# ende76/brotli-rs

Measured on AMD Instinct MI355X. Metric: decompressed MB/s (whole node), alice29x4096 batch, higher is better.
Workload: dtype u8; 1 GPU; 4096 x alice29.txt.compressed per GPU; streams_per_gpu=4096

## Files before the change

### brotli-rs_amd/csrc/brx_hot.S

```

#include "brx_layout.h"
#define RMASK 2047
#define RING BRX_L_RING_BYTES
#define LDS_TM BRX_L_TM
#define LDS_ST BRX_L_ST
#define LDS_MBW BRX_L_MBW
#define LDS_ITAB BRX_L_ITAB
#define LDS_SPARE BRX_L_SPARE
#define LDS_CMH BRX_L_CMH
#define LDS_PAD0 BRX_L_PAD
#define SYMOFF 68
#define INFOOFF 64
#define XLOOP 0x1ffff

#define NPOST s4
#define MA s5
#define MB s6
#define SB s7
#define PFREE s8
#define PBASE s9
#define DTREE s10
#define LINKD s[24:25]
#define XFP s[26:27]
#define LITSYM s28
// ... 10 lines not shown
#define DIST s47
#define RSRC s[48:51]
#define RSRC2 s[16:19]
#define POS s52
#define DSPEC s57
#define SKEW s53
#define VFL s54
#define FLUSHAT s55
#define WINDOW s56
#define INS s92
#define CPY s93
#define MBLEFT s61
#define IZ s64
#define LBLEN s65
#define IBLEN s66
#define DBLEN s67
#define PRIOW s60
#define RUN s68
#define NXT s[58:59]
#define NXTLO s58
#define NXTHI s59
#define WIN s[62:63]
#define WINLO s62
#define WINHI s63
#define MBEND s69
#ifdef BRX_WIN_SGPR
#define SNAV s70
#else
#define SWC s70
#endif
#define DCTX s94
#define HISYM s71
#define MA2 s71
#define BFEB s28
#define CMDW s72
#define EXITC s73
#define IACTAB s[74:75]
#define DICTP s[76:77]
#define LBLEN_REAL s78
#define IBLEN_REAL s79
#define FLAGS s80
#define DCODE s81
#define LINKA s[82:83]
#define T0 s84
#define T1 s85
#define T01 s[84:85]
#define T2 s86
#define T3 s87
#define T4 s88
#define T5 s89
#define T6 s90
#define T7 s91
#define CLEN s96
#if defined(BRX_WIN_SGPR) && !defined(BRX_PROF) && !defined(BRX_NO_SLOTS)
#define BRX_SLOTS
#endif
#ifndef SLOT_OVER
#define SLOT_OVER 11
#endif
#ifndef BRX_PROF
#define LITJ s[20:21]
#define LITJLO s20
#define LITJHI s21
#ifdef BRX_SLOTS
#define BFEBI s29
#define VCCB s[22:23]
#define VCCA s[30:31]
// ... 150 lines not shown
.endm
.macro TAKE_EXTRA dst, base, n, rid, mul=0
    v_bfe_u32 VEX, VWINLO, 0, \n
    .ifnc \mul,0
    v_mad_u32_u24 VEX, VEX, \mul, \base
    .else
    v_add_u32 VEX, \base, VEX
    .endif
    TAKE \n, \rid
    v_readfirstlane_b32 \dst, VEX
.endm
.macro REFILL_CORE
    v_readlane_b32 T0, VCHA, WL
    v_mov_b32 VWLO, VWHI
    s_sub_u32 SWC, SWC, 32
    s_add_u32 WL, WL, 1
    v_mov_b32 VWHI, T0
    s_cmp_lg_u32 WL, WLSTOP
.endm
.macro WIN_INIT lo, hi
    v_mov_b32 VWLO, \lo
    v_mov_b32 VWHI, \hi
    v_alignbit_b32 VWINLO, VWHI, VWLO, SWC
.endm
.macro WIN_ROLLED
.endm
#endif
#ifndef STUB_PAD_NOPS
#define STUB_PAD_NOPS 5
#endif
#ifndef TAIL_PAD_NOPS
#define TAIL_PAD_NOPS 0
#endif
.macro STUB_PAD
#ifndef BRX_WIN_SGPR
    .rept STUB_PAD_NOPS
    s_nop 0
    .endr
#endif
.endm
.macro REFILL_STUB id
.Lrf_stub_\id:
    REFILL_CORE
    s_cbranch_scc1 .Lrf_back_\id
    s_call_b64 LINKA, .Lspecial
    s_branch .Lrf_back_\id
    STUB_PAD
.endm
.macro TO_COUNTS reg, tmp
    v_add_u32 \tmp, -1, VSH
    v_lshrrev_b32 \reg, \tmp, \reg
.endm
.macro SPLIT_TREE lim, base
    v_bfe_i32 \base, \lim, 0, 16
    v_and_b32 \lim, 0xffff0000, \lim
.endm
.macro LOOKUP lim, base
    v_bfrev_b32 VR, WSRC
    v_lshrrev_b32 VU, 1, VR
    v_cmp_lt_u32 vcc, VU, \lim
    s_ff1_i32_b32 CLEN, vcc_lo
    v_readlane_b32 T3, \base, CLEN
    s_sub_u32 T2, 32, CLEN
    v_lshrrev_b32 VI, T2, VR
    v_add_u32 VI, T3, VI
.endm

#ifdef BRX_NO_SPEC
.macro LOOKUP2 lim, base, symbase, scale, rd, off, rid
    v_bfrev_b32 VR, WSRC
    v_lshrrev_b32 VU, 1, VR
    v_cmp_lt_u32 vcc, VU, \lim
    s_ff1_i32_b32 CLEN, vcc_lo
// ... 403 lines not shown
    s_cbranch_scc1 .Lent_multi
    s_bitset1_b32 FLAGS, 3
    s_add_u32 LITSYM, T6, SYMOFF
    v_add_u32 VT0, T6, VLANE4
    ds_read_b32 VLITL, VT0
.Lent_multi:
    s_waitcnt vmcnt(0)
    v_readlane_b32 s36, VCHA, 0
    v_readlane_b32 s37, VCHA, 1
#ifdef BRX_WIN_SGPR
    s_lshr_b64 s[36:37], s[36:37], T3
    s_sub_u32 SNAV, 32, T3
#else
    s_sub_u32 SWC, T3, 32
#endif
    WIN_INIT s36, s37
    s_mov_b32 WL, 2
    s_sub_u32 T0, WSAFE, CBASE
    s_cselect_b32 T0, 0, T0
    s_min_u32 WLSTOP, T0, 64
#ifdef BRX_PROF
    s_mov_b32 s20, 0
    s_mov_b32 s21, 0
    s_mov_b32 s22, 0
    s_mov_b32 s23, 0
    s_mov_b32 s29, 0
    s_mov_b32 s30, 0
    s_mov_b32 s31, 0
    s_memtime s[12:13]
    s_memtime s[16:17]
    s_waitcnt lgkmcnt(0)
#endif
    s_mov_b32 PFREE, 0
    s_mov_b32 PBASE, POS
    s_sub_u32 DCTX, CPY, 2
    s_min_u32 DCTX, DCTX, 3
    s_cmp_lg_u32 IZ, 0
    s_cselect_b32 DCTX, 4, DCTX
    s_mov_b32 T0, 0xc0000000
    s_lshl_b32 DCTX, DCTX, 1
    v_writelane_b32 VDH4, T0, 8
#ifdef BRX_DIST_RESIDENT
    s_call_b64 LINKB, .Lload_dtrees
#endif
    s_mov_b32 EXITC, 1
    s_and_b32 T0, VFL, 0xfffffc00
    s_add_u32 T0, T0, 1024
    s_sub_u32 FLUSHAT, T0, SKEW
    s_waitcnt lgkmcnt(0)
    s_cmp_lt_u32 WLSTOP, 3
    s_cbranch_scc1 .Lexit
    s_and_b32 T0, VFL, 1023
    s_cmp_lg_u32 T0, 0
    s_cbranch_scc1 .Lexit
    SPLIT_TREE VIACL, VIACB
    SPLIT_TREE VLITL, VLITB
    v_lshl_add_u32 VIACB, VIACB, 1, HISYM
    v_lshl_add_u32 VLITB, VLITB, 1, LITSYM
    TO_COUNTS VIACL, VT3
    TO_COUNTS VLITL, VT3
    s_lshr_b32 MA2, MA, 2
    s_mov_b32 BFEB, 0
    s_cmp_eq_u32 SB, 2
    s_cselect_b32 BFEB, 0x20008, BFEB
    s_cmp_eq_u32 MB, 0x1c
    s_cselect_b32 BFEB, 0x3000a, BFEB
#ifndef BRX_PROF
    s_sub_u32 BFEBI, BFEB, 8
    s_cmp_eq_u32 BFEB, 0
    s_cselect_b32 BFEBI, 0, BFEBI
    s_getpc_b64 LITJ
.Llitj_base:
    s_mov_b32 T0, .Llit_entry_g-.Llitj_base
    s_bitcmp1_b32 FLAGS, 5
    s_cselect_b32 T0, .Llit_r_entry_mx-.Llitj_base, T0
    s_cselect_b32 T1, 0x1c, -1
    s_cmp_eq_u32 T1, MB
    s_cselect_b32 T0, .Llit_r_entry_m3-.Llitj_base, T0
#ifdef BRX_SLOTS
    s_bitcmp1_b32 FLAGS, 6
    s_cselect_b32 T0, .Llit_r_entry_sx-.Llitj_base, T0
    s_cselect_b32 T1, 0x1c, -1
    s_cmp_eq_u32 T1, MB
    s_cselect_b32 T0, .Llit_r_entry_s3-.Llitj_base, T0
#endif
    s_bitcmp1_b32 FLAGS, 3
    s_cselect_b32 T0, .Lhave_lits1-.Llitj_base, T0
    s_add_u32 LITJLO, LITJLO, T0
    s_addc_u32 LITJHI, LITJHI, 0
#endif
    s_mov_b32 MAXA, 0
    s_mov_b64 exec, XLOOP
    s_branch .Lr1
// ... 67 lines not shown
    s_waitcnt lgkmcnt(0)
    v_readlane_b32 DCODE, VS, CLEN
    s_cmp_lt_i32 DCODE, 0
    s_cbranch_scc1 .Ldist_ring
    s_and_b32 T1, DCODE, 31
#ifdef BRX_WIN_SGPR
    s_lshr_b32 T2, DCODE, 5
    TAKE_EXTRA DIST, T2, T1, 6, NPOST
#else
    v_lshrrev_b32 VT0, 5, DCODE
    TAKE_EXTRA DIST, VT0, T1, 6, NPOST
#endif
.Ldist_push:
    PROF_MARK s30
    s_cmp_gt_u32 DIST, MAXA
    s_cbranch_scc1 .Ldict_check
.Ldist_push_ok:
    v_mov_b32_dpp VRING, VRING row_shr:1 row_mask:0xf bank_mask:0xf
    v_writelane_b32 VRING, DIST, 0

.Lcopy:
#ifndef BRX_NO_SPEC
    LOOKUP2F_EARLY VIACL, VIACB, 1, ds_read_u16
#endif
    s_bfm_b64 exec, CPY, PFREE
    s_add_u32 PFREE, PFREE, CPY
    s_min_u32 T0, DIST, 63
    s_cmp_gt_u32 PFREE, T0
    s_cbranch_scc1 .Lcopy_slow_undo
    s_sub_u32 T2, PBASE, DIST
    s_cmp_gt_u32 DIST, RING
    s_cbranch_scc0 .Lcopy_near
    v_add_u32 VT0, T2, VLANE
    buffer_load_ubyte VPEND, VT0, RSRC, 0 offen
    s_mov_b64 exec, XLOOP
    s_add_u32 POS, POS, CPY
.Lcopy_tail_pre:
    s_cmp_ge_u32 POS, MBEND
    s_cbranch_scc0 .Lcmd_pre
    s_branch .Lcopy_end
.Lcopy_tail:
.Lflush_back_cmd:
    s_cmp_ge_u32 POS, MBEND
    s_cbranch_scc0 .Lcmd
.Lcopy_end:
    s_cmp_eq_u32 POS, MBEND
    s_cbranch_scc0 .Lcopy_overrun
    s_mov_b32 INS, 0
    s_branch .Lexit
.Lcopy_overrun:
    s_sub_u32 POS, POS, CPY
    s_sub_u32 PFREE, PFREE, CPY
    s_branch .Lx_r2

.Lcopy_near:
    s_add_u32 T2, T2, SKEW
    v_add_u32 VT0, T2, VLANE
    v_and_b32 VT0, RMASK, VT0
    ds_read_u8 VPEND, VT0
    s_mov_b64 exec, XLOOP
    s_add_u32 POS, POS, CPY
    s_cmp_ge_u32 POS, MBEND
    s_cbranch_scc0 .Lcmd_pre
    s_branch .Lcopy_end

#ifdef BRX_DIST_RESIDENT
.Ldist_other:
    s_add_u32 T0, DCTX, 16
    s_bitcmp1_b32 DSPEC, T0
    s_cbranch_scc1 .Ldist_special
    s_sub_u32 DBLEN, DBLEN, 1
    s_cbranch_scc1 .Lx_dist_switch
.Ldist_ticked:
    v_bfrev_b32 VR, WSRC
    v_lshrrev_b32 VI, VSH, VR
    s_set_gpr_idx_on DCTX, 6
    v_cmp_lt_u32 vcc, VI, VDTREES
    v_lshl_add_u32 VI, VI, 2, VDTREES1
    s_set_gpr_idx_off
    ds_read_b32 VS, VI
    s_ff1_i32_b32 CLEN, vcc_lo
    TAKE CLEN, 15
    s_branch .Ldist_have
#endif
.Ldist_special:
#ifdef BRX_DIST_RESIDENT
    v_readlane_b32 DTREE, VDH4, DCTX
#endif
    s_bitcmp1_b32 DTREE, 30
    s_cbranch_scc0 .Ldist_single
.Ldist_zero:
    v_readlane_b32 DIST, VRING, 0
    s_cmp_gt_u32 DIST, MAXA
    s_cbranch_scc0 .Lcopy
    s_min_u32 MAXA, POS, WINDOW
    s_cmp_gt_u32 DIST, MAXA
    s_cbranch_scc0 .Lcopy
// ... 49 lines not shown
    s_call_b64 LINKB, .Lsw_L
    s_branch \again
\flush_stub:
    s_call_b64 LINKC, .Lflush
    s_cmp_lg_u32 INS, 0
    s_cbranch_scc1 \again
    s_branch .Lafter_lits
.Lrf_stub_\id:
    REFILL_CORE
    s_cbranch_scc1 .Lrf_back_\id
    s_add_u32 INS, INS, RUN
    s_add_u32 LBLEN, LBLEN, RUN
    s_sub_u32 POS, POS, RUN
    s_mov_b32 RUN, 0
    s_call_b64 LINKA, .Lspecial
    s_branch .Lrf_back_\id
    STUB_PAD
.endm

.macro LIT_RUN_FAST_STUB id, general_id
.Lrf_stub_\id:
    REFILL_CORE
    s_cbranch_scc1 .Lrf_back_\id
    s_mov_b32 INS, RUN
    s_add_u32 LBLEN, LBLEN, RUN
    s_sub_u32 POS, POS, RUN
    s_mov_b32 RUN, 0
    s_call_b64 LINKA, .Lspecial
    s_branch .Lrf_back_\general_id
    STUB_PAD
.endm

.macro LAND_BODY pbase=1
    s_add_u32 T6, PBASE, SKEW
    s_bfm_b64 exec, PFREE, 0
    v_add_u32 VT1, T6, VLANE
    v_and_b32 VT1, RMASK, VT1
    PROF_WAIT_VM
    s_waitcnt vmcnt(0) lgkmcnt(0)
    ds_write_b8 VT1, VPEND
    s_mov_b64 exec, XLOOP
    s_mov_b32 PFREE, 0
    .if \pbase
    s_mov_b32 PBASE, POS
    .endif
.endm
#ifndef BRX_WIN_SGPR
.macro LAND_BODY_CTX v
    s_add_u32 T6, PBASE, SKEW
    s_bfm_b64 exec, PFREE, 0
    v_add_u32 VT1, T6, VLANE
    v_and_b32 VT1, RMASK, VT1
    PROF_WAIT_VM
    s_waitcnt vmcnt(0) lgkmcnt(0)
    ds_write_b8 VT1, VPEND
    ds_read_u8 VT0, VPEND offset:LDS_ITAB
    s_waitcnt lgkmcnt(0)
.ifc \v,m3
    v_bfe_u32 VT3, VT0, 2, 3
    v_lshlrev_b32 VT2, 3, VT3
.else
    v_and_b32 VT3, MB, VT0
    v_lshrrev_b32 VT2, 2, VT0
.endif
    s_sub_u32 T4, PFREE, 1
    s_add_u32 T0, POS, SKEW
    v_or_b32_dpp VT2, VT3, VT2 wave_shr:1 row_mask:0xf bank_mask:0xf
    s_mov_b64 exec, XLOOP
    s_mov_b32 PFREE, 0
.endm
#endif
.Lhave_lits:
    s_sub_u32 MBLEFT, MBEND, POS
    s_cmp_gt_u32 INS, MBLEFT
    s_cbranch_scc1 .Lexit
#ifndef BRX_PROF
    s_setpc_b64 LITJ
.Llit_entry_g:
#endif
    s_bitcmp1_b32 FLAGS, 3
    s_cbranch_scc1 .Lhave_lits1
    s_call_b64 LINKB, .Lland_ctx
    s_bitcmp1_b32 FLAGS, 5
    s_cbranch_scc1 .Llit_r_start
// ... 47 lines not shown
.Lflush_stub_lit\sfx:
    s_call_b64 LINKC, .Lflush
    s_branch .Lflush_back_lit\sfx
.endm
    LIT_LOOP _u, 0, 4
    LIT_LOOP _m, 1, 8
#ifdef BRX_PROF
.Llit_r_start:
    v_lshrrev_b32 VT0, 2, VC
    v_lshrrev_b32 VT1, 2, VB4
    s_nop 0
    v_readfirstlane_b32 T4, VT0
    v_readfirstlane_b32 T5, VT1
.Llit_r_go:
.macro LIT_R_BODY rid
    v_readlane_b32 T6, VCMAP, T4
    LOOKUP2X \rid
    s_waitcnt lgkmcnt(0)
    v_readlane_b32 T0, VS, CLEN
    s_bfe_u32 T1, T0, 0x6000a
    s_and_b32 T1, T1, MA2
    v_mov_b32 VE, T0
    ds_write_b8 VPA, VE
    v_add_u32 VPA, 1, VPA
    s_or_b32 T4, T1, T5
    s_bfe_u32 T5, T0, BFEB
.endm
    LIT_RUN_FAST .Llit_r_run
.Llit_rf:
    LIT_R_BODY 10
    s_sub_u32 RUN, RUN, 1
    s_cbranch_scc0 .Llit_rf
.Lafter_lits_fast:
    s_mov_b32 PBASE, POS
    s_cmp_eq_u32 POS, MBEND
    s_cbranch_scc0 .Lno_lits
    s_branch .Lexit
.Llit_r_run:
    LIT_RUN_SETUP .Lflush_stub_lit_r, .Llsw_9
.Llit_r:
    LIT_R_BODY 9
    s_sub_u32 RUN, RUN, 1
    s_cbranch_scc0 .Llit_r
    LIT_RUN_END .Llit_r_run, .Lflush_stub_lit_r
    LIT_RUN_STUBS 9, .Llit_r_run, .Lflush_stub_lit_r
    LIT_RUN_FAST_STUB 10, 9
#else
.macro LIT_CTX_RING_BYTES
    v_add_u32 VT0, -1, VPA
    v_add_u32 VT1, -2, VPA
    v_and_b32 VT0, RMASK, VT0
    v_and_b32 VT1, RMASK, VT1
    ds_read_u8 VT0, VT0
    ds_read_u8 VT1, VT1
    s_waitcnt lgkmcnt(0)
    ds_read_u8 VT3, VT0 offset:LDS_ITAB
    ds_read_u8 VT4, VT1 offset:LDS_ITAB
    s_waitcnt lgkmcnt(0)
    v_readfirstlane_b32 T6, VT3
    v_readfirstlane_b32 T7, VT4
.endm
.macro LIT_CTX_ENTRY v
.Llit_r_entry_\v:
    s_cmp_eq_u32 PFREE, 0
    s_cbranch_scc1 .Llit_r_entry_nopend_\v
#ifdef BRX_CTX_RING
    LAND_BODY 0
// ... 39 lines not shown
.macro LIT_CTX_ENTRY_AUX v
#ifndef BRX_CTX_RING
.Llit_r_entry_ring_\v:
    s_add_u32 T6, POS, SKEW
    v_bfe_u32 VPA, T6, 0, 11
    LIT_CTX_RING_BYTES
#ifdef BRX_WIN_SGPR
    s_branch .Llit_r_ctx_have_\v
#else
    LIT_CTX_FROM_INFO \v
    s_branch .Llit_r_go_\v
#endif
#endif
.Llit_r_entry_nopend_\v:
    s_cmp_lt_u32 POS, 2
    s_cbranch_scc0 .Llit_r_entry_ring_\v
    s_call_b64 LINKB, .Lland_ctx
.ifc \v,mx
.Llit_r_start:
.endif
    v_lshrrev_b32 VT0, 2, VC
    v_lshrrev_b32 VT1, 2, VB4
    s_nop 0
    v_readfirstlane_b32 T4, VT0
    v_readfirstlane_b32 T5, VT1
    s_branch .Llit_r_go_\v
.endm
.macro LIT_R_HEAD rid
    v_readlane_b32 T6, VCMAP, T4
    LOOKUP2X \rid
    s_waitcnt lgkmcnt(0)
    v_readlane_b32 T0, VS, CLEN
.endm
.macro LIT_R_STORE
    v_mov_b32 VE, T0
    ds_write_b8 VPA, VE
    v_add_u32 VPA, 1, VPA
.endm
.macro LIT_R_BODY_M3 rid, cur, prev
    LIT_R_HEAD \rid
    s_bfe_u32 \cur, T0, 0x3000d
    s_lshl3_add_u32 T4, \cur, \prev
    LIT_R_STORE
.endm
.macro LIT_R_BODY_MX rid
    LIT_R_HEAD \rid
    s_bfe_u32 T1, T0, 0x6000a
    s_or_b32 T4, T1, T5
    LIT_R_STORE
    s_bfe_u32 T5, T0, BFEB
.endm
.macro LIT_RF_STUB id, back_id
.Lrf_stub_\id:
    REFILL_CORE
    s_cbranch_scc1 .Lrf_back_\id
    s_add_u32 INS, INS, RUN
    s_add_u32 LBLEN, LBLEN, RUN
    s_sub_u32 POS, POS, RUN
    s_mov_b32 RUN, 0
    s_call_b64 LINKA, .Lspecial
    s_branch .Lrf_back_\back_id
    STUB_PAD
.endm
.macro LIT_RUN_TAIL_FAST
    s_mov_b32 PBASE, POS
    s_cmp_eq_u32 POS, MBEND
    s_cbranch_scc0 .Lno_lits
    s_branch .Lexit
.endm
.macro LIT_RUN_AUX v
.Llsw_\v:
    s_call_b64 LINKB, .Lsw_L
    s_branch .Llit_r_run_\v
.Lflush_stub_lit_r_\v:
    s_call_b64 LINKC, .Lflush
    s_cmp_lg_u32 INS, 0
    s_cbranch_scc1 .Llit_r_run_\v
    s_branch .Lafter_lits
.endm
    LIT_CTX_ENTRY m3
    LIT_RUN_FAST .Llit_r_run_m3
.Llit_rf_m3:
    LIT_R_BODY_M3 40, T7, T5
    s_sub_u32 RUN, RUN, 1
    s_cbranch_scc1 .Lafter_lits_fast_m3
    LIT_R_BODY_M3 41, T5, T7
    s_sub_u32 RUN, RUN, 1
    s_cbranch_scc0 .Llit_rf_m3
.Lafter_lits_fast_m3:
    LIT_RUN_TAIL_FAST
.Llit_r_run_m3:
    LIT_RUN_SETUP .Lflush_stub_lit_r_m3, .Llsw_m3
.Llit_r_m3:
    LIT_R_BODY_M3 42, T7, T5
    s_sub_u32 RUN, RUN, 1
    s_cbranch_scc1 .Llit_r_m3_odd
    LIT_R_BODY_M3 43, T5, T7
    s_sub_u32 RUN, RUN, 1
    s_cbranch_scc0 .Llit_r_m3
.Llit_r_m3_end:
    LIT_RUN_END .Llit_r_run_m3, .Lflush_stub_lit_r_m3
.Llit_r_m3_odd:
    s_mov_b32 T5, T7
    s_branch .Llit_r_m3_end
    LIT_RUN_AUX m3
    LIT_CTX_ENTRY_AUX m3
    LIT_RF_STUB 40, 42
    LIT_RF_STUB 41, 43
    LIT_RF_STUB 42, 42
    LIT_RF_STUB 43, 43
    LIT_CTX_ENTRY mx
    LIT_RUN_FAST .Llit_r_run_mx
.Llit_rf_mx:
    LIT_R_BODY_MX 44
    s_sub_u32 RUN, RUN, 1
    s_cbranch_scc0 .Llit_rf_mx
    LIT_RUN_TAIL_FAST
.Llit_r_run_mx:
    LIT_RUN_SETUP .Lflush_stub_lit_r_mx, .Llsw_mx
.Llit_r_mx:
    LIT_R_BODY_MX 45
    s_sub_u32 RUN, RUN, 1
    s_cbranch_scc0 .Llit_r_mx
    LIT_RUN_END .Llit_r_run_mx, .Lflush_stub_lit_r_mx
    LIT_RUN_AUX mx
    LIT_CTX_ENTRY_AUX mx
    LIT_RF_STUB 44, 45
    LIT_RF_STUB 45, 45
#ifdef BRX_SLOTS
.macro SL_COMPARE vs, vccp
    v_bfrev_b32 VR, WINLO
    v_lshrrev_b32 VI, VSH, VR
    v_cmp_lt_u32 \vccp, VI, VQL
    v_lshl_add_u32 VI, VI, 1, VQB
    ds_read_u16 \vs, VI
.endm
.macro SL_SELECT vccp, rid, miss
    v_readlane_b32 T6, VSLOT, T4
    s_bitcmp1_b32 T6, 7
    s_cbranch_scc1 \miss
    s_lshr_b64 T01, \vccp, T6
    s_ff1_i32_b32 CLEN, T0
    s_add_u32 T6, T6, CLEN
    TAKE CLEN, \rid
.endm
.macro SL_FINISH_M3 vs, cnt, cur, prev
    s_waitcnt lgkmcnt(\cnt)
    v_readlane_b32 T0, \vs, T6
    s_bfe_u32 \cur, T0, 0x3000d
    s_lshl3_add_u32 T4, \cur, \prev
    v_writelane_b32 VLITS, T0, m0
.endm
.macro SL_FINISH_MX vs, cnt
    s_waitcnt lgkmcnt(\cnt)
    v_readlane_b32 T0, \vs, T6
    s_bfe_u32 T1, T0, 0x6000a
    s_or_b32 T4, T1, T5
    s_bfe_u32 T5, T0, BFEB
    v_writelane_b32 VLITS, T0, m0
.endm
.macro SL_RF_STUB id
// ... 93 lines not shown
    SL_RF_STUB 50
    SL_RF_STUB 51
    LIT_CTX_ENTRY sx
    SL_RUN sx
.Lsl_a_sx:
    SL_SELECT VCCA, 52, .Lsl_miss_a_sx
    s_sub_u32 m0, m0, 1
    s_cbranch_scc1 .Lsl_last_a_sx
    SL_COMPARE VSB, VCCB
    SL_FINISH_MX VSA, 1
.Lsl_b_sx:
    SL_SELECT VCCB, 53, .Lsl_miss_b_sx
    s_sub_u32 m0, m0, 1
    s_cbranch_scc1 .Lsl_last_b_sx
    SL_COMPARE VSA, VCCA
    SL_FINISH_MX VSB, 1
    s_branch .Lsl_a_sx
.Lsl_last_a_sx:
    SL_FINISH_MX VSA, 0
    s_branch .Lsl_end_sx
.Lsl_last_b_sx:
    SL_FINISH_MX VSB, 0
    SL_RUN_END sx
    SL_MISS sx, a, VSA, VCCA
    SL_MISS sx, b, VSB, VCCB
    LIT_RUN_AUX sx
    LIT_CTX_ENTRY_AUX sx
    SL_RF_STUB 52
    SL_RF_STUB 53
#endif
#endif
.Lafter_lits:
    s_mov_b32 INS, 0
    s_mov_b32 PBASE, POS
    s_cmp_eq_u32 POS, MBEND
    s_cbranch_scc0 .Lno_lits
    s_branch .Lexit

.Lhave_lits1:
    s_call_b64 LINKB, .Lland
    s_add_u32 T0, POS, SKEW
    v_bfe_u32 VPA, T0, 0, 11
    LIT_RUN_FAST .Llit1_run
    s_branch .Llit1
.Llit1_run:
    LIT_RUN_SETUP .Lflush_stub_lit1, .Llsw_7
#if defined(BRX_PROF) || defined(BRX_NO_SPEC) || defined(BRX_LIT1_SERIAL)
.Llit1:
    LOOKUP2F VLITL, VLITB, 1, ds_read_u16, 7
    s_waitcnt lgkmcnt(0)
    v_readlane_b32 T0, VS, CLEN
    s_nop 1
    v_mov_b32 VE, T0
    ds_write_b8 VPA, VE
    v_add_u32 VPA, 1, VPA
    s_sub_u32 RUN, RUN, 1
    s_cbranch_scc0 .Llit1
    s_cmp_lg_u32 INS, 0
    s_cbranch_scc0 .Lafter_lits
    LIT_RUN_END .Llit1_run, .Lflush_stub_lit1
    LIT_RUN_STUBS 7, .Llit1_run, .Lflush_stub_lit1
#else
.macro LOOKUP1 vs, len, rid
    v_bfrev_b32 VR, WSRC
    v_lshrrev_b32 VI, VSH, VR
    v_cmp_lt_u32 vcc, VI, VLITL
    v_lshl_add_u32 VI, VI, 1, VLITB
// ... 197 lines not shown
    s_cmp_eq_u32 vcc_lo, 1
    s_cbranch_scc0 .Lslot_fill_have
    s_lshr_b32 T0, CLEN, 16
    s_bitset1_b32 T0, 31
    s_branch .Lslot_fill_have
.macro SLOT_REMAP
    v_lshlrev_b32 VCMAP, 1, VT4
    v_mov_b32 VSLOT, 0x80
    .irp sl, 0, 1, 2, 3
    s_bfe_u32 T2, SLOTT, 0x80000 + 8 * \sl
    s_lshl_b32 T2, T2, 1
    v_mov_b32 VT0, 16 * \sl
    v_cmp_eq_u32 vcc, T2, VCMAP
    v_cndmask_b32 VSLOT, VSLOT, VT0, vcc
    .endr
.endm
#endif
.Lent_cmh_far:
    s_bitset1_b32 FLAGS, 7
    DESC_GATHER VT4, VT4, 20, 3, VT0, VT1, vcc
    s_branch .Lent_cmh_have
.Lent_vdh_far:
    s_bitset1_b32 FLAGS, 8
    DESC_GATHER VDH4, VT3, 28, 7, VT0, VT1, vcc
    s_branch .Lent_vdh_have
.Lland:
    s_cmp_eq_u32 PFREE, 0
    s_cbranch_scc1 .Lland_chk
    LAND_BODY
.Lland_chk:
    s_cmp_ge_u32 POS, FLUSHAT
    s_cbranch_scc1 .Lland_flush
    s_setpc_b64 LINKB
.Lland_flush:
    FLUSH_BODY .Lland_flush_loop
    s_setpc_b64 LINKB
.Lland_ctx:
    s_cmp_lt_u32 POS, 2
    s_cbranch_scc1 .Lland_ctx_start
    s_cmp_eq_u32 PFREE, 0
    s_cbranch_scc1 .Lland_ctx_ring
    LAND_BODY
.Lland_ctx_ring:
    s_add_u32 T6, POS, SKEW
    v_bfe_u32 VPA, T6, 0, 11
    v_add_u32 VT0, -1, VPA
    v_add_u32 VT1, -2, VPA
    v_and_b32 VT0, RMASK, VT0
    v_and_b32 VT1, RMASK, VT1
    ds_read_u8 VT0, VT0
    ds_read_u8 VT1, VT1
    s_waitcnt lgkmcnt(0)
.Lland_ctx_have:
    ds_read_u8 VT3, VT0 offset:LDS_ITAB
    ds_read_u8 VT4, VT1 offset:LDS_ITAB
    s_waitcnt lgkmcnt(0)
    v_and_b32 VB4, MB, VT3
    v_lshlrev_b32 VB4, SB, VB4
    v_and_b32 VT4, MB, VT4
    v_lshlrev_b32 VT4, SB, VT4
    v_and_or_b32 VC, VT3, MA, VT4
    ds_read_b32 VH, VC offset:LDS_CMH
    s_setpc_b64 LINKB

.Lland_ctx_start:
    s_add_u32 T6, POS, SKEW
    v_bfe_u32 VPA, T6, 0, 11
    v_mov_b32 VT0, 0
    v_mov_b32 VT1, 0
    s_cmp_eq_u32 POS, 0
    s_cbranch_scc1 .Lland_ctx_have
    s_and_b32 T7, SKEW, RMASK
    v_mov_b32 VT0, T7
    ds_read_u8 VT0, VT0
    s_waitcnt lgkmcnt(0)
    s_branch .Lland_ctx_have

.Lflush:
    s_cmp_eq_u32 PFREE, 0
    s_cbranch_scc1 .Lflush_go
    LAND_BODY
.Lflush_go:
    FLUSH_BODY .Lflush_loop
    s_setpc_b64 LINKC

.Lspecial:
    s_cmp_lg_u32 WL, 64
    s_cbranch_scc1 .Lnear_end
    s_waitcnt vmcnt(0)
    s_mov_b64 exec, -1
    v_mov_b32 VCHA, VCHB
    s_add_u32 CBASE, CBASE, 64
    s_add_u32 T0, CBASE, 64
    v_add_u32 VT4, T0, VLANE
    v_min_u32 VT4, WENDM1, VT4
    v_lshlrev_b32 VT4, 2, VT4
    global_load_dword VCHB, VT4, INP
    s_mov_b64 exec, XLOOP
    s_mov_b32 WL, 0
    WIN_ROLLED
    s_lshr_b32 T0, CBASE, 6
    s_add_u32 T0, T0, PRIOW
    s_and_b32 T0, T0, 3
    s_cmp_lt_u32 T0, 2
    s_cbranch_scc1 .Lprio_01
    s_cmp_eq_u32 T0, 2
    s_cbranch_scc1 .Lprio_2
    s_setprio 3
    s_branch .Lprio_done
.Lprio_2:
    s_setprio 2
    s_branch .Lprio_done
.Lprio_01:
    s_cmp_eq_u32 T0, 0
    s_cbranch_scc1 .Lprio_0
    s_setprio 1
    s_branch .Lprio_done
// ... 46 lines not shown
    s_call_b64 LINKB, .Lland
    s_branch .Lcopy
.Lcopy_odd:
    s_cmp_lt_u32 DIST, CPY
    s_cbranch_scc0 .Lcopy_long

.Lcopy_overlap:
    s_min_u32 T0, MBLEFT, 64
    s_cmp_gt_u32 CPY, T0
    s_cbranch_scc1 .Lcopy_long
    s_call_b64 LINKB, .Lland
    s_mov_b64 exec, -1
    s_sub_u32 T0, CPY, 1
    v_min_u32 VT2, T0, VLANE
    v_mov_b32 VT0, VT2
    .irp k, 5, 4, 3, 2, 1, 0
    s_lshl_b32 T2, DIST, \k
    v_subrev_u32 VT1, T2, VT0
    v_cmp_le_u32 vcc, T2, VT0
    v_cndmask_b32 VT0, VT0, VT1, vcc
    .endr
    s_sub_u32 T1, POS, DIST
    s_add_u32 T1, T1, SKEW
    v_add_u32 VT0, T1, VT0
    v_and_b32 VT0, RMASK, VT0
    ds_read_u8 VT3, VT0
    s_add_u32 T1, POS, SKEW
    v_add_u32 VT0, T1, VT2
    v_and_b32 VT0, RMASK, VT0
    s_waitcnt lgkmcnt(0)
    ds_write_b8 VT0, VT3
    s_mov_b64 exec, XLOOP
    s_add_u32 POS, POS, CPY
    s_mov_b32 PBASE, POS
    s_branch .Lcopy_tail

.macro PERIOD_CHUNK off
    s_min_u32 T0, T5, 64
    s_sub_u32 T1, T0, 1
    v_min_u32 VT2, T1, VLANE
    .if \off
    v_add_u32 VT0, \off, VT2
    .else
    v_mov_b32 VT0, VT2
    .endif
    .irp k, 6, 5, 4, 3, 2, 1, 0
    s_lshl_b32 T2, DIST, \k
    v_subrev_u32 VT1, T2, VT0
    v_cmp_le_u32 vcc, T2, VT0
    v_cndmask_b32 VT0, VT0, VT1, vcc
    .endr
    v_add_u32 VT0, T3, VT0
    v_and_b32 VT0, RMASK, VT0
    ds_read_u8 VT3, VT0
    s_add_u32 T1, POS, SKEW
    v_add_u32 VT0, T1, VT2
    v_and_b32 VT0, RMASK, VT0
    s_waitcnt lgkmcnt(0)
    ds_write_b8 VT0, VT3
    s_add_u32 POS, POS, T0
    s_sub_u32 T5, T5, T0
.endm
#ifndef COPY_NEAR_MAX
#define COPY_NEAR_MAX 8191
#endif
.Lcopy_long:
    s_mov_b32 T0, COPY_NEAR_MAX
    s_cmp_gt_u32 DIST, RING
    s_cselect_b32 T0, 512, T0
    s_min_u32 T0, MBLEFT, T0
    s_cmp_gt_u32 CPY, T0
    s_cbranch_scc1 .Lx_r2
    s_call_b64 LINKB, .Lland
    s_mov_b32 T5, CPY
    s_cmp_lt_u32 DIST, 64
    s_cbranch_scc0 .Lcl_chunk
#ifdef BRX_NO_PERIOD_COPY
    s_branch .Lx_r2
#endif
    s_mov_b64 exec, -1
    s_sub_u32 T3, POS, DIST
    s_add_u32 T3, T3, SKEW
    PERIOD_CHUNK 0
    PERIOD_CHUNK 64
    s_mov_b64 exec, XLOOP
    s_mov_b32 PBASE, POS
    s_flbit_i32_b32 T0, DIST
    s_sub_u32 T0, T0, 25
    s_lshl_b32 DIST, DIST, T0
    s_cmp_ge_u32 POS, FLUSHAT
    s_cbranch_scc0 .Lcp_noflush
    s_call_b64 LINKC, .Lflush
.Lcp_noflush:
    s_cmp_lg_u32 T5, 0
    s_cbranch_scc1 .Lcl_chunk
    s_branch .Lflush_back_cmd
.Lcl_chunk:
    s_mov_b64 exec, -1
    s_min_u32 T0, T5, 64
    s_sub_u32 T1, T0, 1
    v_min_u32 VT1, T1, VLANE
    s_sub_u32 T1, POS, DIST
    s_cmp_gt_u32 DIST, RING
    s_cbranch_scc1 .Lcl_far
    s_add_u32 T1, T1, SKEW
    v_add_u32 VT0, T1, VT1
    v_and_b32 VT0, RMASK, VT0
    ds_read_u8 VT2, VT0
    s_branch .Lcl_have
.Lcl_far:
    v_add_u32 VT0, T1, VT1
    buffer_load_ubyte VT2, VT0, RSRC, 0 offen
.Lcl_have:
    s_add_u32 T1, POS, SKEW
    v_add_u32 VT0, T1, VT1
    v_and_b32 VT0, RMASK, VT0
    s_waitcnt vmcnt(0) lgkmcnt(0)
    ds_write_b8 VT0, VT2
    s_mov_b64 exec, XLOOP
    s_add_u32 POS, POS, T0
    s_sub_u32 T5, T5, T0
    s_mov_b32 PBASE, POS
    s_cmp_ge_u32 POS, FLUSHAT
    s_cbranch_scc0 .Lcl_noflush
    s_call_b64 LINKC, .Lflush
.Lcl_noflush:
    s_cmp_lg_u32 T5, 0
    s_cbranch_scc1 .Lcl_chunk
    s_branch .Lflush_back_cmd

.Ldict_xform:
    s_cmp_gt_u32 T3, 120
    s_cbranch_scc1 .Lx_r2
    s_mul_i32 T4, T3, 20
    s_load_dwordx4 s[12:15], XFP, T4
    s_add_u32 T4, T4, 16
    s_load_dword s97, XFP, T4
    s_waitcnt lgkmcnt(0)
    s_bfe_u32 T1, s97, 0x80010
    s_sub_u32 T4, T1, 1
    s_cmp_lt_u32 T4, 2
    s_cbranch_scc1 .Lxf_land
    s_cmp_gt_u32 PFREE, 23
    s_cbranch_scc0 .Lxf_landed
.Lxf_land:
    s_call_b64 LINKB, .Lland
.Lxf_landed:
    s_and_b32 T2, s97, 0xff
    s_bfe_u32 T3, s97, 0x80008
    s_mov_b32 T5, 0
    s_mov_b32 T7, CPY
    s_cmp_lt_u32 T1, 3
    s_cbranch_scc1 .Lxf_have
    s_cmp_ge_u32 T1, 12
    s_cbranch_scc1 .Lxf_last
// ... 88 lines not shown
    v_mov_b32 VT0, T0
    v_cmp_eq_u32 vcc, T4, VLANE
    v_cndmask_b32 VT0, 0, VT0, vcc
    v_or_b32 VT1, VT1, VT0
    s_cmp_eq_u32 T1, 1
    s_cbranch_scc1 .Lxf_up_done
    s_cmp_lt_u32 T6, CPY
    s_cbranch_scc1 .Lxf_up_loop
.Lxf_up_done:
    v_xor_b32 VT3, VT3, VT1
.Lxf_store:
    v_lshlrev_b32 VT1, 3, VLANE
    v_lshrrev_b64 v[54:55], VT1, s[12:13]
    s_add_u32 T4, POS, SKEW
    v_add_u32 VT0, T4, VLANE
    v_and_b32 VT0, RMASK, VT0
    s_bfm_b64 exec, T2, 0
    ds_write_b8 VT0, v54
    s_mov_b64 exec, -1
    s_add_u32 T4, T4, T2
    v_add_u32 VT0, T4, VLANE
    v_and_b32 VT0, RMASK, VT0
    s_bfm_b64 exec, T7, 0
    ds_write_b8 VT0, VT3
    s_mov_b64 exec, -1
    s_add_u32 T4, T4, T7
    v_lshrrev_b64 v[54:55], VT1, s[14:15]
    v_add_u32 VT0, T4, VLANE
    v_and_b32 VT0, RMASK, VT0
    s_bfm_b64 exec, T3, 0
    ds_write_b8 VT0, v54
    s_mov_b64 exec, XLOOP
    s_add_u32 POS, POS, CLEN
    s_mov_b32 PBASE, POS
    s_branch .Lcopy_tail

.Lswitch:
    s_bitcmp1_b32 FLAGS, 0
    s_cbranch_scc1 .Lsw_ret
    v_mov_b32 VT0, T7
    ds_read_b64 v[20:21], VT0 offset:LDS_MBW
    ds_read_b32 v22, VT0 offset:LDS_MBW+8
    ds_read_b64 v[24:25], VT0 offset:LDS_MBW+16
    s_waitcnt lgkmcnt(0)
    v_readfirstlane_b32 s12, v20
    v_readfirstlane_b32 s13, v21
    v_readfirstlane_b32 s14, v22
    v_readfirstlane_b32 s36, v24
    v_readfirstlane_b32 s37, v25
    s_lshl_b32 s36, s36, 2
    s_lshl_b32 s37, s37, 2
    s_add_u32 s36, s36, LDS_TM
    s_add_u32 s37, s37, LDS_TM
    v_add_u32 VT1, s36, VLANE4
    v_add_u32 VT2, s37, VLANE4
    ds_read_b32 VLIM, VT1
    ds_read_b32 v14, VT2
    v_mov_b32 VT1, s36
    v_mov_b32 VT2, s37
    ds_read_b32 VT1, VT1 offset:INFOOFF
    ds_read_b32 VT2, VT2 offset:INFOOFF
    s_waitcnt lgkmcnt(0)
    SPLIT_TREE VLIM, VBASE
    SPLIT_TREE v14, v15
    v_readfirstlane_b32 T2, VT1
    v_readfirstlane_b32 T3, VT2
    s_and_b32 T2, T2, 3
// ... 363 lines not shown
```

Before: 79010 MB/s.

## Keep PBASE in ring-skewed space and pair literal stores with offset writes

PBASE now holds POS+SKEW, so the copy and land paths no longer add SKEW per use. A separate buffer resource with its base pre-adjusted by SKEW keeps far-copy global loads correct. Literal loops in the m3 and mx contexts now issue byte stores with an immediate offset and bump VPA once per pair, which removes one VALU add per literal. DEAD_PAD nops keep code alignment stable. The cost is extra SGPR aliasing (BFEB moved to s58) and more complex refill stubs that must fix VPA on odd exits.

```diff
diff --git a/brotli-rs_amd/csrc/brx_hot.S b/brotli-rs_amd/csrc/brx_hot.S
--- a/brotli-rs_amd/csrc/brx_hot.S
+++ b/brotli-rs_amd/csrc/brx_hot.S
@@ -66,7 +66,18 @@
 #define DCTX s94
 #define HISYM s71
 #define MA2 s71
+#if !defined(BRX_WIN_SGPR) && !defined(BRX_PROF)
+#define BRX_RING_PBASE
+#endif
+#if !defined(BRX_WIN_SGPR) && !defined(BRX_PROF) && !defined(BRX_NO_PAIRS)
+#define BRX_PAIR_STORE
+#endif
+#ifdef BRX_RING_PBASE
+#define BFEB s58
+#define RSRCS s[28:31]
+#else
 #define BFEB s28
+#endif
 #define CMDW s72
 #define EXITC s73
 #define IACTAB s[74:75]
@@ -283,6 +294,13 @@
 #ifndef TAIL_PAD_NOPS
 #define TAIL_PAD_NOPS 0
 #endif
+#ifdef BRX_RING_PBASE
+.macro DEAD_PAD n
+    .rept \n
+    s_nop 0
+    .endr
+.endm
+#endif
 .macro STUB_PAD
 #ifndef BRX_WIN_SGPR
     .rept STUB_PAD_NOPS
@@ -290,6 +308,11 @@
     .endr
 #endif
 .endm
+#ifdef BRX_RING_PBASE
+#define PBASE_AT_POS s_add_u32 PBASE, POS, SKEW
+#else
+#define PBASE_AT_POS s_mov_b32 PBASE, POS
+#endif
 .macro REFILL_STUB id
 .Lrf_stub_\id:
     REFILL_CORE
@@ -759,7 +782,7 @@
     s_waitcnt lgkmcnt(0)
 #endif
     s_mov_b32 PFREE, 0
-    s_mov_b32 PBASE, POS
+    PBASE_AT_POS
     s_sub_u32 DCTX, CPY, 2
     s_min_u32 DCTX, DCTX, 3
     s_cmp_lg_u32 IZ, 0
@@ -786,6 +809,12 @@
     v_lshl_add_u32 VLITB, VLITB, 1, LITSYM
     TO_COUNTS VIACL, VT3
     TO_COUNTS VLITL, VT3
+#ifdef BRX_RING_PBASE
+    s_sub_u32 s28, s48, SKEW
+    s_mov_b32 s29, s49
+    s_add_u32 s30, s50, SKEW
+    s_mov_b32 s31, s51
+#endif
     s_lshr_b32 MA2, MA, 2
     s_mov_b32 BFEB, 0
     s_cmp_eq_u32 SB, 2
@@ -919,7 +948,11 @@
     s_cmp_gt_u32 DIST, RING
     s_cbranch_scc0 .Lcopy_near
     v_add_u32 VT0, T2, VLANE
+#ifdef BRX_RING_PBASE
+    buffer_load_ubyte VPEND, VT0, RSRCS, 0 offen
+#else
     buffer_load_ubyte VPEND, VT0, RSRC, 0 offen
+#endif
     s_mov_b64 exec, XLOOP
     s_add_u32 POS, POS, CPY
 .Lcopy_tail_pre:
@@ -941,7 +974,9 @@
     s_branch .Lx_r2
 
 .Lcopy_near:
+#ifndef BRX_RING_PBASE
     s_add_u32 T2, T2, SKEW
+#endif
     v_add_u32 VT0, T2, VLANE
     v_and_b32 VT0, RMASK, VT0
     ds_read_u8 VPEND, VT0
@@ -950,6 +985,9 @@
     s_cmp_ge_u32 POS, MBEND
     s_cbranch_scc0 .Lcmd_pre
     s_branch .Lcopy_end
+#ifdef BRX_RING_PBASE
+    DEAD_PAD 1
+#endif
 
 #ifdef BRX_DIST_RESIDENT
 .Ldist_other:
@@ -1065,9 +1103,14 @@
 .endm
 
 .macro LAND_BODY pbase=1
+#ifndef BRX_RING_PBASE
     s_add_u32 T6, PBASE, SKEW
     s_bfm_b64 exec, PFREE, 0
     v_add_u32 VT1, T6, VLANE
+#else
+    s_bfm_b64 exec, PFREE, 0
+    v_add_u32 VT1, PBASE, VLANE
+#endif
     v_and_b32 VT1, RMASK, VT1
     PROF_WAIT_VM
     s_waitcnt vmcnt(0) lgkmcnt(0)
@@ -1075,14 +1118,19 @@
     s_mov_b64 exec, XLOOP
     s_mov_b32 PFREE, 0
     .if \pbase
-    s_mov_b32 PBASE, POS
+    PBASE_AT_POS
     .endif
 .endm
 #ifndef BRX_WIN_SGPR
 .macro LAND_BODY_CTX v
+#ifndef BRX_RING_PBASE
     s_add_u32 T6, PBASE, SKEW
     s_bfm_b64 exec, PFREE, 0
     v_add_u32 VT1, T6, VLANE
+#else
+    s_bfm_b64 exec, PFREE, 0
+    v_add_u32 VT1, PBASE, VLANE
+#endif
     v_and_b32 VT1, RMASK, VT1
     PROF_WAIT_VM
     s_waitcnt vmcnt(0) lgkmcnt(0)
@@ -1196,7 +1244,7 @@
     s_sub_u32 RUN, RUN, 1
     s_cbranch_scc0 .Llit_rf
 .Lafter_lits_fast:
-    s_mov_b32 PBASE, POS
+    PBASE_AT_POS
     s_cmp_eq_u32 POS, MBEND
     s_cbranch_scc0 .Lno_lits
     s_branch .Lexit
@@ -1302,6 +1350,7 @@
     s_waitcnt lgkmcnt(0)
     v_readlane_b32 T0, VS, CLEN
 .endm
+#ifndef BRX_PAIR_STORE
 .macro LIT_R_STORE
     v_mov_b32 VE, T0
     ds_write_b8 VPA, VE
@@ -1320,6 +1369,36 @@
     LIT_R_STORE
     s_bfe_u32 T5, T0, BFEB
 .endm
+#define LIT_BODY_M3(rid, cur, prev, half) LIT_R_BODY_M3 rid, cur, prev
+#else
+.macro LIT_R_STORE half
+    v_mov_b32 VE, T0
+    .if \half == 1
+    ds_write_b8 VPA, VE offset:1
+    v_add_u32 VPA, 2, VPA
+    .else
+    ds_write_b8 VPA, VE
+    .if \half == 2
+    v_add_u32 VPA, 1, VPA
+    .endif
+    .endif
+.endm
+.macro LIT_R_BODY_M3 rid, cur, prev, half
+    LIT_R_HEAD \rid
+    s_bfe_u32 \cur, T0, 0x3000d
+    s_lshl3_add_u32 T4, \cur, \prev
+    LIT_R_STORE \half
+.endm
+.macro LIT_R_BODY_MX rid, half
+    LIT_R_HEAD \rid
+    s_bfe_u32 T1, T0, 0x6000a
+    s_or_b32 T4, T1, T5
+    LIT_R_STORE \half
+    s_bfe_u32 T5, T0, BFEB
+.endm
+#define LIT_BODY_M3(rid, cur, prev, half) LIT_R_BODY_M3 rid, cur, prev, half
+#endif
+#ifndef BRX_PAIR_STORE
 .macro LIT_RF_STUB id, back_id
 .Lrf_stub_\id:
     REFILL_CORE
@@ -1332,8 +1411,27 @@
     s_branch .Lrf_back_\back_id
     STUB_PAD
 .endm
+#else
+.macro LIT_RF_STUB id, back_id, pad=STUB_PAD_NOPS, vpa=0
+.Lrf_stub_\id:
+    REFILL_CORE
+    s_cbranch_scc1 .Lrf_back_\id
+    s_add_u32 INS, INS, RUN
+    s_add_u32 LBLEN, LBLEN, RUN
+    s_sub_u32 POS, POS, RUN
+    s_mov_b32 RUN, 0
+    .if \vpa
+    v_add_u32 VPA, 1, VPA
+    .endif
+    s_call_b64 LINKA, .Lspecial
+    s_branch .Lrf_back_\back_id
+    .rept \pad
+    s_nop 0
+    .endr
+.endm
+#endif
 .macro LIT_RUN_TAIL_FAST
-    s_mov_b32 PBASE, POS
+    PBASE_AT_POS
     s_cmp_eq_u32 POS, MBEND
     s_cbranch_scc0 .Lno_lits
     s_branch .Lexit
@@ -1348,13 +1446,16 @@
     s_cbranch_scc1 .Llit_r_run_\v
     s_branch .Lafter_lits
 .endm
+#ifdef BRX_RING_PBASE
+    DEAD_PAD 1
+#endif
     LIT_CTX_ENTRY m3
     LIT_RUN_FAST .Llit_r_run_m3
 .Llit_rf_m3:
-    LIT_R_BODY_M3 40, T7, T5
+    LIT_BODY_M3(40, T7, T5, 0)
     s_sub_u32 RUN, RUN, 1
     s_cbranch_scc1 .Lafter_lits_fast_m3
-    LIT_R_BODY_M3 41, T5, T7
+    LIT_BODY_M3(41, T5, T7, 1)
     s_sub_u32 RUN, RUN, 1
     s_cbranch_scc0 .Llit_rf_m3
 .Lafter_lits_fast_m3:
@@ -1362,25 +1463,36 @@
 .Llit_r_run_m3:
     LIT_RUN_SETUP .Lflush_stub_lit_r_m3, .Llsw_m3
 .Llit_r_m3:
-    LIT_R_BODY_M3 42, T7, T5
+    LIT_BODY_M3(42, T7, T5, 0)
     s_sub_u32 RUN, RUN, 1
     s_cbranch_scc1 .Llit_r_m3_odd
-    LIT_R_BODY_M3 43, T5, T7
+    LIT_BODY_M3(43, T5, T7, 1)
     s_sub_u32 RUN, RUN, 1
     s_cbranch_scc0 .Llit_r_m3
 .Llit_r_m3_end:
     LIT_RUN_END .Llit_r_run_m3, .Lflush_stub_lit_r_m3
 .Llit_r_m3_odd:
     s_mov_b32 T5, T7
+#ifdef BRX_PAIR_STORE
+    v_add_u32 VPA, 1, VPA
+#endif
     s_branch .Llit_r_m3_end
     LIT_RUN_AUX m3
     LIT_CTX_ENTRY_AUX m3
     LIT_RF_STUB 40, 42
     LIT_RF_STUB 41, 43
     LIT_RF_STUB 42, 42
+#ifndef BRX_PAIR_STORE
     LIT_RF_STUB 43, 43
+#ifdef BRX_RING_PBASE
+    DEAD_PAD 1
+#endif
+#else
+    LIT_RF_STUB 43, 43, STUB_PAD_NOPS + 2
+#endif
     LIT_CTX_ENTRY mx
     LIT_RUN_FAST .Llit_r_run_mx
+#ifndef BRX_PAIR_STORE
 .Llit_rf_mx:
     LIT_R_BODY_MX 44
     s_sub_u32 RUN, RUN, 1
@@ -1393,10 +1505,34 @@
     s_sub_u32 RUN, RUN, 1
     s_cbranch_scc0 .Llit_r_mx
     LIT_RUN_END .Llit_r_run_mx, .Lflush_stub_lit_r_mx
+#else
+.Llit_rf_mx:
+    LIT_R_BODY_MX 44, 0
+    s_sub_u32 RUN, RUN, 1
+    s_cbranch_scc1 .Lafter_lits_fast_mx
+    LIT_R_BODY_MX 46, 1
+    s_sub_u32 RUN, RUN, 1
+    s_cbranch_scc0 .Llit_rf_mx
+.Lafter_lits_fast_mx:
+    LIT_RUN_TAIL_FAST
+.Llit_r_run_mx:
+    LIT_RUN_SETUP .Lflush_stub_lit_r_mx, .Llsw_mx
+.Llit_r_mx:
+    LIT_R_BODY_MX 45, 2
+    s_sub_u32 RUN, RUN, 1
+    s_cbranch_scc0 .Llit_r_mx
+    LIT_RUN_END .Llit_r_run_mx, .Lflush_stub_lit_r_mx
+#endif
     LIT_RUN_AUX mx
     LIT_CTX_ENTRY_AUX mx
+#ifndef BRX_PAIR_STORE
     LIT_RF_STUB 44, 45
     LIT_RF_STUB 45, 45
+#else
+    LIT_RF_STUB 44, 45
+    LIT_RF_STUB 45, 45
+    LIT_RF_STUB 46, 45, STUB_PAD_NOPS, 1
+#endif
 #ifdef BRX_SLOTS
 .macro SL_COMPARE vs, vccp
     v_bfrev_b32 VR, WINLO
@@ -1556,7 +1692,7 @@
 #endif
 .Lafter_lits:
     s_mov_b32 INS, 0
-    s_mov_b32 PBASE, POS
+    PBASE_AT_POS
     s_cmp_eq_u32 POS, MBEND
     s_cbranch_scc0 .Lno_lits
     s_branch .Lexit
@@ -1820,6 +1956,9 @@
     s_cmp_ge_u32 POS, FLUSHAT
     s_cbranch_scc1 .Lland_flush
     s_setpc_b64 LINKB
+#ifdef BRX_RING_PBASE
+    DEAD_PAD 1
+#endif
 .Lland_flush:
     FLUSH_BODY .Lland_flush_loop
     s_setpc_b64 LINKB
@@ -1850,6 +1989,9 @@
     v_and_or_b32 VC, VT3, MA, VT4
     ds_read_b32 VH, VC offset:LDS_CMH
     s_setpc_b64 LINKB
+#ifdef BRX_RING_PBASE
+    DEAD_PAD 1
+#endif
 
 .Lland_ctx_start:
     s_add_u32 T6, POS, SKEW
@@ -1871,6 +2013,9 @@
 .Lflush_go:
     FLUSH_BODY .Lflush_loop
     s_setpc_b64 LINKC
+#ifdef BRX_RING_PBASE
+    DEAD_PAD 1
+#endif
 
 .Lspecial:
     s_cmp_lg_u32 WL, 64
@@ -1983,7 +2128,7 @@
     ds_write_b8 VT0, VT3
     s_mov_b64 exec, XLOOP
     s_add_u32 POS, POS, CPY
-    s_mov_b32 PBASE, POS
+    PBASE_AT_POS
     s_branch .Lcopy_tail
 
 .macro PERIOD_CHUNK off
@@ -2035,7 +2180,7 @@
     PERIOD_CHUNK 0
     PERIOD_CHUNK 64
     s_mov_b64 exec, XLOOP
-    s_mov_b32 PBASE, POS
+    PBASE_AT_POS
     s_flbit_i32_b32 T0, DIST
     s_sub_u32 T0, T0, 25
     s_lshl_b32 DIST, DIST, T0
@@ -2071,7 +2216,7 @@
     s_mov_b64 exec, XLOOP
     s_add_u32 POS, POS, T0
     s_sub_u32 T5, T5, T0
-    s_mov_b32 PBASE, POS
+    PBASE_AT_POS
     s_cmp_ge_u32 POS, FLUSHAT
     s_cbranch_scc0 .Lcl_noflush
     s_call_b64 LINKC, .Lflush
@@ -2226,7 +2371,7 @@
     ds_write_b8 VT0, v54
     s_mov_b64 exec, XLOOP
     s_add_u32 POS, POS, CLEN
-    s_mov_b32 PBASE, POS
+    PBASE_AT_POS
     s_branch .Lcopy_tail
 
 .Lswitch:
```

Result: no change. 79300 MB/s, median of 6 (+0.4%).
